# qinzheng93/GeoTransformer

Hardware: NVIDIA H100
Metric: point-cloud pairs/sec (3DMatch-shape synth) (higher is better)
Workload: dtype f32

## Files before the change

__graft_entry__.py:

```python
import os
import subprocess
import sys

ROOT = os.path.dirname(os.path.abspath(__file__))
if ROOT not in sys.path:
    sys.path.insert(0, ROOT)


def build():
    jobs = str(os.cpu_count() or 4)
    subprocess.check_call(['make', '-C', os.path.join(ROOT, 'geotransformer_b200', 'csrc'), '-j', jobs])
    subprocess.check_call(['make', '-C', os.path.join(ROOT, 'oracle'), 'all'])
    from oracle import normals_oracle, voxel_oracle
    voxel_oracle.build()
    normals_oracle.build()
    import geotransformer_b200
    from geotransformer_b200 import _lib
    _lib.lib()


def smoke():
    import numpy as np
    import torch
    from geotransformer_b200.config import make_cfg
    from geotransformer_b200.model import create_model
    from geotransformer_b200.synth import make_pair
    from geotransformer_b200.utils.data import registration_collate_fn_stack_mode
    from geotransformer_b200.weights import synthetic_state_dict
    from oracle import geo_oracle as G

    assert torch.cuda.is_available(), 'smoke() needs a GPU'
    torch.cuda.set_device(0)
    cfg = make_cfg('3dmatch')
    model = create_model(cfg)
    model.load_state_dict(synthetic_state_dict(model, 7351), strict=True)
    model = model.cuda().eval()
    pair = make_pair('demo2k', 0)
    dd = {k: pair[k] for k in ('ref_points', 'src_points', 'ref_feats', 'src_feats', 'transform')}
# ... 50 lines not shown
```

geotransformer_b200/_lib.py:

```python
import ctypes
import os
import threading

import torch

_HERE = os.path.dirname(os.path.abspath(__file__))
LIB_PATH = os.path.join(_HERE, 'libgeob200.so')
_lib = None

c_void_p, c_int64, c_int32, c_float, c_double, c_size_t, c_int = (
    ctypes.c_void_p, ctypes.c_int64, ctypes.c_int32, ctypes.c_float, ctypes.c_double, ctypes.c_size_t, ctypes.c_int)

SIGNATURES = {}


def _sig(name, restype, *argtypes):
    SIGNATURES[name] = (restype, list(argtypes))


P, I64, I32, F, D, SZ = c_void_p, c_int64, c_int32, c_float, c_double, c_size_t
_sig('geob200_last_error', ctypes.c_char_p)
_sig('geob200_launch_count', ctypes.c_uint64)
_sig('geob200_grid_subsample_workspace_bytes', SZ, I64, I64)
_sig('geob200_grid_subsample', c_int, P, I64, P, I64, F, P, P, P, SZ, P)
_sig('geob200_radius_search_workspace_bytes', SZ, I64, I64, I64)
_sig('geob200_radius_search', c_int, P, I64, P, I64, P, P, I64, F, I64, P, P, P, P, SZ, P)

_sig('geob200_neighbor_histogram', c_int, P, I64, I64, I64, I64, P, P)
_sig('geob200_neighbor_histogram_batched', c_int, P, P, P, I64, I64, I64, I64, P, P, P, P)
_sig('geob200_voxel_down_sample_workspace_bytes', SZ, I64, I64)
_sig('geob200_voxel_down_sample', c_int, P, P, I64, P, I64, D, P, P, P, P, SZ, P)
_sig('geob200_estimate_normals_workspace_bytes', SZ, I64, I64)
_sig('geob200_estimate_normals', c_int, P, I64, P, I64, I64, D, P, P, P, P, P, SZ, P)
_sig('geob200_regularize_normals', c_int, P, P, I64, c_int, c_int, P, P)
_sig('geob200_kernel_point_optimize', c_int, P, I64, I64, ctypes.c_uint64, D, P, P, P)
_sig('geob200_kernel_point_instances', c_int, P, I64, P, P, I64, ctypes.c_uint64, P, P)
_sig('geob200_kpconv_workspace_bytes', SZ, I64)
_sig('geob200_kpconv', c_int, P, P, P, P, I64, I64, I64, P, I64, P, P, I64, I64, F, P, P, SZ, P)
_sig('geob200_kpconv_tc_workspace_bytes', SZ, I64, I64, I64)
_sig('geob200_kpconv_tc', c_int, P, P, P, P, I64, I64, I64, P, I64, P, P, I64, I64, F, P, P, SZ, P)
_sig('geob200_set_linear_mode', None, c_int)
_sig('geob200_linear', c_int, P, I64, P, P, P, I64, I64, I64, I64, c_int, P)
_sig('geob200_split_tf32', c_int, P, I64, I64, I64, P, P)
_sig('geob200_linear_batched', c_int, P, I64, I64, P, I64, I64, P, I64, P, I64, I64, I64, I64, I64, I64, c_int, P)
_sig('geob200_group_norm_workspace_bytes', SZ, I64)
_sig('geob200_group_norm', c_int, P, I64, I64, I64, P, P, F, P, c_int, F, P, P, SZ, P)
_sig('geob200_fused_group_norm_workspace_bytes', SZ, I64, I64, I64)
_sig('geob200_linear_group_norm', c_int, P, I64, P, P, I64, I64, I64, I64, P, P, F, P, c_int, F, P, P, P, SZ, P)
_sig('geob200_kpconv_group_norm', c_int, P, P, P, P, I64, I64, I64, P, I64, P, P, I64, I64, F, I64, P, P, F, c_int, F, P, P, P, SZ,
     P, SZ, P)
_sig('geob200_group_norm_batched', c_int, P, I64, I64, I64, P, P, F, P, c_int, F, P, P, SZ, P, I64, P)
_sig('geob200_linear_group_norm_batched', c_int, P, I64, P, P, I64, I64, I64, I64, P, P, F, P, c_int, F, P, P, P, SZ, P, I64, P)
_sig('geob200_maxpool', c_int, P, P, I64, I64, I64, I64, P, P)
_sig('geob200_upsample_concat', c_int, P, P, I64, I64, P, I64, I64, I64, P, P)
_sig('geob200_kpconv_backward_workspace_bytes', SZ, I64, I64, I64, I64, I64)
_sig('geob200_kpconv_backward', c_int, P, P, P, P, I64, I64, I64, P, I64, P, I64, I64, F, P, P, P, P, P, SZ, P)
_sig('geob200_linear_backward_workspace_bytes', SZ, I64, I64, I64, c_int)
_sig('geob200_linear_backward', c_int, P, I64, P, P, I64, I64, I64, P, P, P, P, P, SZ, P)
_sig('geob200_group_norm_backward_batched_workspace_bytes', SZ, I64, I64, I64, I64)
_sig('geob200_group_norm_backward_batched', c_int, P, P, I64, I64, I64, P, F, c_int, F, P, P, P, P, P, P, SZ, P, I64, P)
_sig('geob200_maxpool_backward_batched_workspace_bytes', SZ, I64, I64, I64, I64)
_sig('geob200_maxpool_backward_batched', c_int, P, P, I64, I64, I64, I64, P, I64, P, P, P, P, SZ, P)
_sig('geob200_upsample_concat_backward_workspace_bytes', SZ, I64, I64)
# ... 177 lines not shown
```

geotransformer_b200/csrc/kpconv.cu:

```cuda
#include "common.cuh"
#include "geob200.h"
#include "kpconv.cuh"

namespace geob200 {

constexpr int TQ = 32;
constexpr int CC = 32;

__global__ void __launch_bounds__(256) kpconv_c1_kernel(const float* __restrict__ feats, const float* __restrict__ q_pts,
                                                        const float* __restrict__ s_pts, const long long* __restrict__ nbr,
                                                        int H, const float* __restrict__ kp, const float* __restrict__ W,
                                                        const float* __restrict__ bias, float sigma, int Ns, int M, int Cout,
                                                        float* __restrict__ out) {
    __shared__ float kp_s[KP * 3];
    __shared__ float wk_s[16][KP_PAD];
    __shared__ float np_s[16];
    if (threadIdx.x < KP * 3) kp_s[threadIdx.x] = kp[threadIdx.x];
    __syncthreads();
    const int lane = threadIdx.x & 31, warp = threadIdx.x >> 5;
    const int sub = lane >> 4, sl = lane & 15;
    const int slot = warp * 2 + sub;
    const int m = blockIdx.x * 16 + slot;
    const bool live = m < M;
    float acc[KP];
// ... 28 lines not shown
    }
    __syncwarp();
    if (!live) return;
    for (int c = sl; c < Cout; c += 16) {
        float o = 0.f;
#pragma unroll
        for (int k = 0; k < KP; ++k) o = fmaf(wk_s[slot][k], W[k * Cout + c], o);
        o = o / np_s[slot];
        if (bias != nullptr) o += bias[c];
        out[(long long)m * Cout + c] = o;
    }
}

__global__ void __launch_bounds__(256) row_positive_kernel(const float* __restrict__ x, int N, int C, unsigned char* __restrict__ pos) {
    const int lane = threadIdx.x & 31;
    const int n = blockIdx.x * 8 + (threadIdx.x >> 5);
    if (n >= N) return;
    float s = 0.f;
    for (int c = lane; c < C; c += 32) s += x[(long long)n * C + c];
    s = warp_sum(s);
    if (lane == 0) pos[n] = (s > 0.f) ? 1 : 0;
}

template <int CPL>
__global__ void __launch_bounds__(256, 4) kpconv_gather_kernel(const float* __restrict__ feats, const unsigned char* __restrict__ pos,
                                                            const float* __restrict__ q_pts, const float* __restrict__ s_pts,
                                                            const long long* __restrict__ nbr, int H, const float* __restrict__ kp,
                                                            float sigma, int Ns, int M, int Cin, float* __restrict__ wf,
                                                            float* __restrict__ inv_count) {
    __shared__ float infl[8][32][KP_PAD];
    __shared__ int sidx[8][32];
    __shared__ float kp_s[KP * 3];
    const int lane = threadIdx.x & 31, warp = threadIdx.x >> 5;
    if (threadIdx.x < KP * 3) kp_s[threadIdx.x] = kp[threadIdx.x];
    __syncthreads();
    const int m = blockIdx.x * 8 + warp;
    if (m >= M) return;
    const float qx = q_pts[3ll * m], qy = q_pts[3ll * m + 1], qz = q_pts[3ll * m + 2];
    int npos = 0;
    for (int c0 = 0; c0 < Cin; c0 += 32 * CPL) {
        float acc[CPL][KP];
#pragma unroll
        for (int p = 0; p < CPL; ++p)
#pragma unroll
            for (int k = 0; k < KP; ++k) acc[p][k] = 0.f;
        for (int h0 = 0; h0 < H; h0 += 32) {
            const int h = h0 + lane;
            const long long idx = (h < H) ? nbr[(long long)m * H + h] : (long long)Ns;
            float w[KP];
            int id = 0;
            if (idx < Ns) {
                id = (int)idx;
                influence15(kp_s, s_pts[3 * idx] - qx, s_pts[3 * idx + 1] - qy, s_pts[3 * idx + 2] - qz, 0.f, sigma, w);
                if (c0 == 0) npos += pos[idx];
            } else {
#pragma unroll
                for (int k = 0; k < KP; ++k) w[k] = 0.f;
            }
            __syncwarp();
#pragma unroll
            for (int k = 0; k < KP; ++k) infl[warp][lane][k] = w[k];
            infl[warp][lane][KP] = 0.f;
            sidx[warp][lane] = id;
            __syncwarp();
            const int hn = min(32, H - h0);
            for (int hb = 0; hb < hn; hb += 8) {
                float f[8][CPL];
#pragma unroll
                for (int u = 0; u < 8; ++u)
#pragma unroll
                    for (int p = 0; p < CPL; ++p)
                        f[u][p] = __ldg(feats + (long long)sidx[warp][(hb + u) & 31] * Cin + c0 + 32 * p + lane);
#pragma unroll
                for (int u = 0; u < 8; ++u) {
                    if (hb + u < hn) {
                        const float4* iv = reinterpret_cast<const float4*>(&infl[warp][hb + u][0]);
                        const float4 a0 = iv[0], a1 = iv[1], a2 = iv[2], a3 = iv[3];
                        const float wv[16] = {a0.x, a0.y, a0.z, a0.w, a1.x, a1.y, a1.z, a1.w, a2.x, a2.y, a2.z, a2.w, a3.x, a3.y, a3.z, a3.w};
#pragma unroll
                        for (int p = 0; p < CPL; ++p)
#pragma unroll
                            for (int k = 0; k < KP; ++k) acc[p][k] = fmaf(wv[k], f[u][p], acc[p][k]);
                    }
                }
            }
        }
#pragma unroll
        for (int p = 0; p < CPL; ++p) {
            float* wrow = wf + (long long)m * (KP * Cin) + c0 + 32 * p + lane;
#pragma unroll
            for (int k = 0; k < KP; ++k) wrow[(long long)k * Cin] = acc[p][k];
        }
    }
#pragma unroll
    for (int o = 16; o > 0; o >>= 1) npos += __shfl_xor_sync(0xffffffffu, npos, o);
    if (lane == 0) inv_count[m] = 1.0f / (float)max(npos, 1);
}

static void launch_kpconv_gather(const float* s_feats, const unsigned char* pos, const float* q_points, const float* s_points,
                                 const long long* neighbors, int n_neighbors, const float* kernel_points, float sigma, int n_support,
                                 int n_query, int c_in, float* wf, float* inv_count, cudaStream_t st) {
    const unsigned grid = (unsigned)((n_query + 7) / 8);
    if (c_in % 64 == 0)
        kpconv_gather_kernel<2><<<grid, 256, 0, st>>>(s_feats, pos, q_points, s_points, neighbors, n_neighbors, kernel_points, sigma,
                                                     n_support, n_query, c_in, wf, inv_count);
    else
        kpconv_gather_kernel<1><<<grid, 256, 0, st>>>(s_feats, pos, q_points, s_points, neighbors, n_neighbors, kernel_points, sigma,
                                                     n_support, n_query, c_in, wf, inv_count);
}

void kpconv_gather(const float* s_feats, const float* q_points, const float* s_points, const long long* neighbors, int n_neighbors,
                   const float* kernel_points, float sigma, int n_support, int n_query, int c_in, unsigned char* pos, float* wf,
                   float* inv_count, cudaStream_t st) {
    row_positive_kernel<<<(unsigned)((n_support + 7) / 8), 256, 0, st>>>(s_feats, n_support, c_in, pos);
    launch_kpconv_gather(s_feats, pos, q_points, s_points, neighbors, n_neighbors, kernel_points, sigma, n_support, n_query, c_in, wf,
                         inv_count, st);
    count_launches(2);
}

template <int RC>
__global__ void __launch_bounds__(256) kpconv_kernel(const float* __restrict__ feats, const unsigned char* __restrict__ pos,
                                                     const float* __restrict__ q_pts, const float* __restrict__ s_pts,
                                                     const long long* __restrict__ nbr, int H, const float* __restrict__ kp,
                                                     const float* __restrict__ W, const float* __restrict__ bias, float sigma,
                                                     int Ns, int M, int Cin, int Cout, float* __restrict__ out) {
    const int col0 = blockIdx.y * (RC * 32);
    extern __shared__ float smem[];
    float* wf = smem;
    float* infl = wf + TQ * KP * CC;
    int* sidx = (int*)(infl + 8 * 32 * KP_PAD);
    float* npos_s = (float*)(sidx + 8 * 32);
    float* kp_s = npos_s + TQ;
    const int lane = threadIdx.x & 31, warp = threadIdx.x >> 5;
    if (threadIdx.x < KP * 3) kp_s[threadIdx.x] = kp[threadIdx.x];
    __syncthreads();
    const int m0 = blockIdx.x * TQ;

    float acc_out[4][RC];
#pragma unroll
    for (int r = 0; r < 4; ++r)
// ... 616 lines not shown
    const long long idx = up[(long long)m * up_stride];
    float* yr = y + (long long)m * (C1 + C2);
    for (int c = lane; c < C1; c += 32) yr[c] = (idx < Ns) ? x[idx * C1 + c] : 0.f;
    if (skip != nullptr)
        for (int c = lane; c < C2; c += 32) yr[C1 + c] = skip[(long long)m * C2 + c];
}

}

using namespace geob200;

namespace geob200 {
int linear_tc(const float* x, int64_t ldx, const float* w, int64_t ldw, const float* w_img, const float* bias, const float* row_scale, float* y, int64_t ldy,
              int64_t m, int64_t n, int64_t k, int relu, cudaStream_t st, const GnFuse* gn = nullptr);
static int g_linear_mode = 1;
}

extern "C" {

void geob200_set_linear_mode(int mode) { g_linear_mode = mode; }

size_t geob200_kpconv_workspace_bytes(int64_t n_support) { return (size_t)n_support + 256; }

size_t geob200_kpconv_tc_workspace_bytes(int64_t n_query, int64_t n_support, int64_t c_in) {
    return align_up((size_t)n_support, 256) + align_up((size_t)n_query * 4, 256) + (size_t)n_query * KP * (size_t)c_in * 4 + 1024;
}

int geob200_kpconv_tc(const float* s_feats, const float* q_points, const float* s_points, const int64_t* neighbors, int64_t n_query,
                      int64_t n_support, int64_t n_neighbors, const float* kernel_points, int64_t n_kernel, const float* weights_t,
                      const float* bias, int64_t c_in, int64_t c_out, float sigma, float* out, void* workspace, size_t workspace_bytes,
                      void* stream) {
    return geob200::kpconv_tc_impl(s_feats, q_points, s_points, neighbors, n_query, n_support, n_neighbors, kernel_points, n_kernel,
                                   weights_t, nullptr, bias, c_in, c_out, sigma, out, workspace, workspace_bytes, stream);
}
}

namespace geob200 {
int kpconv_tc_impl(const float* s_feats, const float* q_points, const float* s_points, const int64_t* neighbors, int64_t n_query,
                   int64_t n_support, int64_t n_neighbors, const float* kernel_points, int64_t n_kernel, const float* weights_t,
                   const float* w_img, const float* bias, int64_t c_in, int64_t c_out, float sigma, float* out, void* workspace,
                   size_t workspace_bytes, void* stream) {
    cudaStream_t st = (cudaStream_t)stream;
    GEOB_REQUIRE(n_kernel == KP, "kpconv_tc: kernel_size %lld unsupported", (long long)n_kernel);
    GEOB_REQUIRE(n_query > 0 && n_support > 0 && n_neighbors > 0, "kpconv_tc: empty input");
    GEOB_REQUIRE(c_in % 32 == 0 && c_out % 16 == 0 && c_out >= 32 && (c_out <= 128 || c_out % 128 == 0) && n_query >= 64,
                 "kpconv_tc: unsupported shape (%lld -> %lld, %lld queries)", (long long)c_in, (long long)c_out, (long long)n_query);
    GEOB_REQUIRE(workspace_bytes >= geob200_kpconv_tc_workspace_bytes(n_query, n_support, c_in), "kpconv_tc: workspace too small");
    Arena ar(workspace, workspace_bytes);
    unsigned char* pos = ar.take<unsigned char>(n_support);
    float* inv_count = ar.take<float>(n_query);
    float* wf = ar.take<float>((size_t)n_query * KP * c_in);
    row_positive_kernel<<<(unsigned)((n_support + 7) / 8), 256, 0, st>>>(s_feats, (int)n_support, (int)c_in, pos);
    launch_kpconv_gather(s_feats, pos, q_points, s_points, (const long long*)neighbors, (int)n_neighbors, kernel_points, sigma,
                         (int)n_support, (int)n_query, (int)c_in, wf, inv_count, st);
    GEOB_CHECK_LAUNCH();
    count_launches(2);
    const int rc = linear_tc(wf, KP * c_in, weights_t, KP * c_in, w_img, bias, inv_count, out, c_out, n_query, c_out, KP * c_in, 0, st);
    GEOB_REQUIRE(rc == 0, "kpconv_tc: tensor-core GEMM rejected the shape");
    return 0;
}

int linear_img(const float* x, int64_t ldx, const float* weight, const float* w_img, const float* bias, float* y, int64_t ldy,
               int64_t m, int64_t n, int64_t k, int relu, void* stream) {
    if (g_linear_mode == 1 && m > 0 && n > 0 && k > 0) {
        const int rc = linear_tc(x, ldx, weight, k, w_img, bias, nullptr, y, ldy, m, n, k, relu, (cudaStream_t)stream);
        if (rc <= 0) return rc;
    }
    return geob200_linear(x, ldx, weight, bias, y, ldy, m, n, k, relu, stream);
}
}

extern "C" {

int geob200_kpconv(const float* s_feats, const float* q_points, const float* s_points, const int64_t* neighbors,
                   int64_t n_query, int64_t n_support, int64_t n_neighbors, const float* kernel_points, int64_t n_kernel,
                   const float* weights, const float* bias, int64_t c_in, int64_t c_out, float sigma, float* out,
                   void* workspace, size_t workspace_bytes, void* stream) {
    cudaStream_t st = (cudaStream_t)stream;
    GEOB_REQUIRE(n_kernel == KP, "kpconv: kernel_size %lld unsupported (all shipped models use 15)", (long long)n_kernel);
// ... 248 lines not shown
namespace geob200 {
int kpconv_group_norm_impl(const float* s_feats, const float* q_points, const float* s_points, const int64_t* neighbors,
                           int64_t n_query, int64_t n_support, int64_t n_neighbors, const float* kernel_points, int64_t n_kernel,
                           const float* weights_t, const float* bias, int64_t c_in, int64_t c_out, float sigma, int64_t groups,
                           const float* gamma, const float* beta, float eps, int leaky, float slope, float* pre_norm, float* y,
                           void* gn_workspace, size_t gn_workspace_bytes, void* workspace, size_t workspace_bytes, void* stream,
                           const GnSeg* seg, const float* w_img) {
    cudaStream_t st = (cudaStream_t)stream;
    const int64_t np = (seg != nullptr && seg->n_pairs > 1) ? seg->n_pairs : 1;
    GEOB_REQUIRE(n_kernel == KP, "kpconv_group_norm: kernel_size %lld unsupported", (long long)n_kernel);
    GEOB_REQUIRE(n_query > 0 && n_support > 0 && n_neighbors > 0, "kpconv_group_norm: empty input");
    GEOB_REQUIRE(c_in % 32 == 0 && c_out % 16 == 0 && c_out >= 32 && (c_out <= 128 || c_out % 128 == 0) && n_query >= 64,
                 "kpconv_group_norm: unsupported shape (%lld -> %lld, %lld queries)", (long long)c_in, (long long)c_out,
                 (long long)n_query);
    GEOB_REQUIRE(groups > 0 && c_out % groups == 0, "kpconv_group_norm: bad group count");
    GEOB_REQUIRE(gn_workspace_bytes >= (np > 1 ? fused_group_norm_workspace_bytes_batched(n_query, c_out, groups, np)
                                               : geob200_fused_group_norm_workspace_bytes(n_query, c_out, groups)),
                 "kpconv_group_norm: GroupNorm workspace too small");
    GEOB_REQUIRE(workspace_bytes >= geob200_kpconv_tc_workspace_bytes(n_query, n_support, c_in), "kpconv_group_norm: workspace too small");
    Arena ar(workspace, workspace_bytes);
    unsigned char* pos = ar.take<unsigned char>(n_support);
    float* inv_count = ar.take<float>(n_query);
    float* wf = ar.take<float>((size_t)n_query * KP * c_in);
    row_positive_kernel<<<(unsigned)((n_support + 7) / 8), 256, 0, st>>>(s_feats, (int)n_support, (int)c_in, pos);
    launch_kpconv_gather(s_feats, pos, q_points, s_points, (const long long*)neighbors, (int)n_neighbors, kernel_points, sigma,
                         (int)n_support, (int)n_query, (int)c_in, wf, inv_count, st);
    GEOB_CHECK_LAUNCH();
    count_launches(2);
    const GnWs w = gn_carve(gn_workspace, gn_workspace_bytes, groups, np);
    GnFuse gn{(int)groups, 0, w.partial};
    int rc = linear_tc(wf, KP * c_in, weights_t, KP * c_in, w_img, bias, inv_count, pre_norm, c_out, n_query, c_out, KP * c_in, 0, st, &gn);
    if (rc < 0) return rc;
    if (rc == 0) {
        if (np > 1) {
            launch_gn_seg_apply(pre_norm, w, gamma, beta, nullptr, y, n_query, c_out, groups, eps, leaky, slope, *seg, st);
        } else {
            launch_gn_apply(pre_norm, w, gamma, beta, nullptr, y, n_query, c_out, groups, eps, leaky, slope, st);
            count_launches(2);
        }
        GEOB_CHECK_LAUNCH();
        return 0;
    }
    rc = linear_tc(wf, KP * c_in, weights_t, KP * c_in, w_img, bias, inv_count, pre_norm, c_out, n_query, c_out, KP * c_in, 0, st);
    GEOB_REQUIRE(rc == 0, "kpconv_group_norm: tensor-core GEMM rejected the shape");
    return group_norm_impl(pre_norm, n_query, c_out, groups, gamma, beta, eps, nullptr, leaky, slope, y, gn_workspace, gn_workspace_bytes,
                           stream, seg);
}
}

namespace geob200 {
int make_seg(GnSeg* g, int64_t n_pairs, const int64_t* cloud_rows_h, int64_t n_rows, const char* what) {
// ... 86 lines not shown
```

geotransformer_b200/csrc/kpconv.cuh:

```cuda
#pragma once
#include "common.cuh"

namespace geob200 {

constexpr int KP = 15;
constexpr int KP_PAD = 16;

__device__ __forceinline__ void influence15(const float* __restrict__ kp_s, float rx, float ry, float rz, float inv_dummy,
                                            float sigma, float* w) {
#pragma unroll
    for (int k = 0; k < KP; ++k) {
        const float dx = rx - kp_s[3 * k], dy = ry - kp_s[3 * k + 1], dz = rz - kp_s[3 * k + 2];
        const float sq = __fadd_rn(__fadd_rn(__fmul_rn(dx, dx), __fmul_rn(dy, dy)), __fmul_rn(dz, dz));
        w[k] = fmaxf(1.0f - sqrtf(sq) / sigma, 0.0f);
    }
    (void)inv_dummy;
}

__device__ __forceinline__ int cloud_of(const int* start, int n_clouds, int row) {
    int lo = 0, hi = n_clouds;
    while (hi - lo > 1) {
        const int mid = (lo + hi) >> 1;
        if (start[mid] <= row) lo = mid; else hi = mid;
    }
    return lo;
}

int make_seg(GnSeg* g, int64_t n_pairs, const int64_t* cloud_rows_h, int64_t n_rows, const char* what);

void kpconv_gather(const float* s_feats, const float* q_points, const float* s_points, const long long* neighbors, int n_neighbors,
                   const float* kernel_points, float sigma, int n_support, int n_query, int c_in, unsigned char* pos, float* wf,
                   float* inv_count, cudaStream_t st);

size_t atb_bytes(int64_t M, int64_t ka, int64_t n);
void atb(const float* A, long long lda, const float* B, long long ldb, const float* s, int64_t M, int64_t ka, int64_t n, float* C,
         float* part, cudaStream_t st);

}
```

geotransformer_b200/csrc/kpconv_grad.cu:

```cuda
#include "common.cuh"
#include "geob200.h"
#include "kpconv.cuh"

namespace geob200 {

__global__ void __launch_bounds__(1024) exclusive_scan_kernel(const int* __restrict__ cnt, int n, int* __restrict__ off);

struct IndexTable {
    const long long* idx;
    long long ld;
    int rows, cols, n_support;
    __device__ __forceinline__ int target(int e) const {
        const int m = e / cols, h = e - m * cols;
        const long long v = idx[(long long)m * ld + h];
        return (v >= 0 && v < n_support) ? (int)v : -1;
    }
};

__global__ void __launch_bounds__(256) csr_count_kernel(IndexTable t, int* __restrict__ cnt) {
    const int e = blockIdx.x * blockDim.x + threadIdx.x;
    if (e >= t.rows * t.cols) return;
    const int s = t.target(e);
    if (s >= 0) atomicAdd(&cnt[s], 1);
}
// ... 456 lines not shown
    GEOB_REQUIRE(n_query > 0 && n_support > 0 && n_neighbors > 0 && c_out > 0, "kpconv_backward: empty input");
    GEOB_REQUIRE(c_in == 1 || c_in % 32 == 0, "kpconv_backward: c_in %lld must be 1 or a multiple of 32", (long long)c_in);
    GEOB_REQUIRE(n_query * n_neighbors < (1ll << 31) && n_query * KP * c_in < (1ll << 40), "kpconv_backward: neighbour table too large");
    GEOB_REQUIRE(s_feats != nullptr && q_points != nullptr && s_points != nullptr && neighbors != nullptr && kernel_points != nullptr &&
                 grad_out != nullptr && (grad_feats == nullptr || weights != nullptr), "kpconv_backward: null input");
    GEOB_REQUIRE(workspace != nullptr &&
                 workspace_bytes >= geob200_kpconv_backward_workspace_bytes(n_query, n_support, n_neighbors, c_in, c_out),
                 "kpconv_backward: workspace too small");
    const int64_t ka = KP * c_in;
    Arena ar(workspace, workspace_bytes);
    unsigned char* pos = ar.take<unsigned char>(n_support);
    float* inv_count = ar.take<float>(n_query);
    float* wf = ar.take<float>((size_t)n_query * ka);
    float* part = ar.take<float>(atb_bytes(n_query, ka, c_out) / 4 + atb_bytes(n_query, 1, c_out) / 4 + 1);
    const long long* nbr = (const long long*)neighbors;
    if (grad_bias != nullptr) atb(nullptr, 0, grad_out, c_out, nullptr, n_query, 1, c_out, grad_bias, part, st);
    if (grad_weights != nullptr || grad_feats != nullptr) {
        if (c_in == 1) {
            kpconv_c1_wf_kernel<<<(unsigned)((n_query + 15) / 16), 256, 0, st>>>(s_feats, q_points, s_points, nbr, (int)n_neighbors,
                                                                                 kernel_points, sigma, (int)n_support, (int)n_query, wf,
                                                                                 inv_count);
            count_launches(1);
        } else {
            kpconv_gather(s_feats, q_points, s_points, nbr, (int)n_neighbors, kernel_points, sigma, (int)n_support, (int)n_query, (int)c_in,
                          pos, wf, inv_count, st);
        }
    }
    if (grad_weights != nullptr) atb(wf, ka, grad_out, c_out, inv_count, n_query, ka, c_out, grad_weights, part, st);
    if (grad_feats != nullptr) {
        const int rc = linear_img(grad_out, c_out, weights, nullptr, nullptr, wf, ka, n_query, ka, c_out, 0, stream);
        if (rc != 0) return rc;
        Csr csr;
        const IndexTable t{nbr, n_neighbors, (int)n_query, (int)n_neighbors, (int)n_support};
        if (build_csr(t, ar, &csr, st)) return -1;
        kpconv_dx_kernel<<<(unsigned)((n_support + 7) / 8), 256, 0, st>>>(wf, inv_count, q_points, s_points, kernel_points, sigma,
                                                                          (int)n_neighbors, (int)n_support, (int)c_in, csr.off,
                                                                          csr.sorted, grad_feats);
        count_launches(1);
    }
    GEOB_REQUIRE(ar.ok(), "kpconv_backward: workspace accounting error");
    GEOB_CHECK_LAUNCH();
    return 0;
}

size_t geob200_linear_backward_workspace_bytes(int64_t m, int64_t n, int64_t k, int relu) {
    return atb_bytes(m, n, k) + atb_bytes(m, 1, n) + (relu ? align_up((size_t)m * n * 4, 256) : 0) + 1024;
}

// ... 131 lines not shown
```

geotransformer_b200/functional.py:

```python
import ctypes
import math

import torch

from . import _lib as L

_f32, _i64, _u8, _i32 = torch.float32, torch.int64, torch.uint8, torch.int32

GSE_MODE = 5
GSE_TABLE_INV_STEP = 256
GSE_TABLE_D_MAX = 96.0

EVENTS = None


class _timed:
    def __init__(self, name):
        self.name = name

    def __enter__(self):
        if EVENTS is not None:
            self.s = torch.cuda.Event(enable_timing=True)
            self.e = torch.cuda.Event(enable_timing=True)
            self.s.record()
# ... 47 lines not shown
def _kpconv(s_feats, q_points, s_points, neighbor_indices, kernel_points, weights, bias, sigma, weights_t=None):
    s_feats, weights, bias = _detach(s_feats), _detach(weights), _detach(bias)
    _f(s_feats, 's_feats'); _f(q_points, 'q_points'); _f(s_points, 's_points')
    L.require_cuda(neighbor_indices, 'neighbor_indices', _i64)
    m, h = neighbor_indices.shape
    ns = s_points.shape[0]
    k, cin, cout = weights.shape
    out = torch.empty((m, cout), dtype=_f32, device=s_feats.device)
    lib = L.lib()
    if (KPCONV_MODE == 'tc' and cin % 32 == 0 and cout % 16 == 0 and cout >= 32 and (cout <= 128 or cout % 128 == 0) and m >= 64):
        if weights_t is None:
            weights_t = weights.reshape(k * cin, cout).t().contiguous()
        ws = L.workspace(lib.geob200_kpconv_tc_workspace_bytes(m, ns, cin), s_feats.device, 'kpconv_tc')
        L.check(lib.geob200_kpconv_tc(s_feats.data_ptr(), q_points.data_ptr(), s_points.data_ptr(), neighbor_indices.data_ptr(), m, ns,
                                      h, kernel_points.data_ptr(), k, weights_t.data_ptr(), L.ptr(bias), cin, cout, float(sigma),
                                      out.data_ptr(), ws.data_ptr(), ws.numel(), L.stream_ptr()), 'kpconv_tc')
        return out
    ws = L.workspace(lib.geob200_kpconv_workspace_bytes(ns), s_feats.device, 'kpconv')
    L.check(lib.geob200_kpconv(s_feats.data_ptr(), q_points.data_ptr(), s_points.data_ptr(),
                               neighbor_indices.data_ptr(), m, ns, h, kernel_points.data_ptr(), k,
                               weights.data_ptr(), L.ptr(bias), cin, cout, float(sigma), out.data_ptr(),
                               ws.data_ptr(), ws.numel(), L.stream_ptr()), 'kpconv')
    return out


def kpconv_backward(s_feats, q_points, s_points, neighbor_indices, kernel_points, weights, sigma, grad_out, need_feats=True,
                    need_weights=True, need_bias=True):
    for t, name in ((s_feats, 's_feats'), (q_points, 'q_points'), (s_points, 's_points'), (kernel_points, 'kernel_points'),
                    (weights, 'weights'), (grad_out, 'grad_out')):
        _f(_detach(t), name)
    L.require_cuda(neighbor_indices, 'neighbor_indices', _i64)
    s_feats, weights = _detach(s_feats), _detach(weights)
    m, h = neighbor_indices.shape
    ns = s_points.shape[0]
    k, cin, cout = weights.shape
    if tuple(grad_out.shape) != (m, cout) or tuple(s_feats.shape) != (ns, cin):
        raise RuntimeError(f'kpconv_backward: grad_out must be ({m}, {cout}) and s_feats ({ns}, {cin})')
    dev = s_feats.device
    gf = torch.empty((ns, cin), dtype=_f32, device=dev) if need_feats else None
    gw = torch.empty((k, cin, cout), dtype=_f32, device=dev) if need_weights else None
    gb = torch.empty((cout,), dtype=_f32, device=dev) if need_bias else None
    lib = L.lib()
    ws = L.workspace(lib.geob200_kpconv_backward_workspace_bytes(m, ns, h, cin, cout), dev, 'kpconv_backward')
    L.check(lib.geob200_kpconv_backward(s_feats.data_ptr(), q_points.data_ptr(), s_points.data_ptr(), neighbor_indices.data_ptr(), m, ns, h,
                                        kernel_points.data_ptr(), k, weights.data_ptr(), cin, cout, float(sigma), grad_out.data_ptr(),
                                        L.ptr(gf), L.ptr(gw), L.ptr(gb), ws.data_ptr(), ws.numel(), L.stream_ptr()), 'kpconv_backward')
# ... 2360 lines not shown
```

include/geob200.h:

```cpp
#ifndef GEOB200_H
#define GEOB200_H

#include <stddef.h>
#include <stdint.h>

#ifdef __cplusplus
extern "C" {
#endif

const char* geob200_last_error(void);
uint64_t geob200_launch_count(void);


size_t geob200_grid_subsample_workspace_bytes(int64_t n_points, int64_t batch);
int geob200_grid_subsample(const float* points, int64_t n_points, const int64_t* lengths_h, int64_t batch, float voxel,
                           float* s_points, int64_t* s_lengths, void* workspace, size_t workspace_bytes, void* stream);

size_t geob200_radius_search_workspace_bytes(int64_t n_query, int64_t n_support, int64_t batch);
int geob200_radius_search(const float* q_points, int64_t n_query, const float* s_points, int64_t n_support,
                          const int64_t* q_lengths_h, const int64_t* s_lengths_h, int64_t batch, float radius,
                          int64_t width, int64_t* out, int32_t* counts, int32_t* max_count, void* workspace,
                          size_t workspace_bytes, void* stream);

int geob200_neighbor_histogram(const int64_t* neighbors, int64_t n_rows, int64_t width, int64_t n_support, int64_t hist_n,
// ... 24 lines not shown
                             size_t workspace_bytes, void* stream);
int geob200_regularize_normals(const void* points, const void* normals, int64_t n, int fp64, int positive, double* out, void* stream);


#define GEOB200_KP_MAX_POINTS 30
int geob200_kernel_point_optimize(const double* init, int64_t num_kernels, int64_t num_points, uint64_t seed, double ratio,
                                  double* points, int32_t* info, void* stream);

int geob200_kernel_point_instances(const double* disposition, int64_t num_points, const double* radii, const int64_t* layer_ids,
                                   int64_t num_layers, uint64_t seed, float* out, void* stream);


size_t geob200_kpconv_workspace_bytes(int64_t n_support);
int geob200_kpconv(const float* s_feats, const float* q_points, const float* s_points, const int64_t* neighbors,
                   int64_t n_query, int64_t n_support, int64_t n_neighbors, const float* kernel_points, int64_t n_kernel,
                   const float* weights, const float* bias, int64_t c_in, int64_t c_out, float sigma, float* out,
                   void* workspace, size_t workspace_bytes, void* stream);

size_t geob200_kpconv_tc_workspace_bytes(int64_t n_query, int64_t n_support, int64_t c_in);
int geob200_kpconv_tc(const float* s_feats, const float* q_points, const float* s_points, const int64_t* neighbors, int64_t n_query,
                      int64_t n_support, int64_t n_neighbors, const float* kernel_points, int64_t n_kernel, const float* weights_t,
                      const float* bias, int64_t c_in, int64_t c_out, float sigma, float* out, void* workspace, size_t workspace_bytes,
                      void* stream);

int geob200_split_tf32(const float* w, int64_t ld, int64_t n, int64_t k, float* out, void* stream);

void geob200_set_linear_mode(int mode);
int geob200_linear(const float* x, int64_t ldx, const float* weight, const float* bias, float* y, int64_t ldy, int64_t m,
                   int64_t n, int64_t k, int relu, void* stream);
int geob200_linear_batched(const float* x, int64_t ldx, int64_t stride_x, const float* weight, int64_t ldw, int64_t stride_w,
                           const float* bias, int64_t stride_b, float* y, int64_t ldy, int64_t stride_y, int64_t m, int64_t n,
                           int64_t k, int64_t batch, int relu, void* stream);

size_t geob200_group_norm_workspace_bytes(int64_t groups);
int geob200_group_norm(const float* x, int64_t n_rows, int64_t channels, int64_t groups, const float* gamma,
                       const float* beta, float eps, const float* residual, int leaky, float slope, float* y,
                       void* workspace, size_t workspace_bytes, void* stream);

size_t geob200_fused_group_norm_workspace_bytes(int64_t n_rows, int64_t channels, int64_t groups);
int geob200_linear_group_norm(const float* x, int64_t ldx, const float* weight, const float* bias, int64_t m, int64_t n, int64_t k,
                              int64_t groups, const float* gamma, const float* beta, float eps, const float* residual, int leaky,
                              float slope, float* pre_norm, float* y, void* workspace, size_t workspace_bytes, void* stream);
int geob200_kpconv_group_norm(const float* s_feats, const float* q_points, const float* s_points, const int64_t* neighbors,
                              int64_t n_query, int64_t n_support, int64_t n_neighbors, const float* kernel_points, int64_t n_kernel,
                              const float* weights_t, const float* bias, int64_t c_in, int64_t c_out, float sigma, int64_t groups,
                              const float* gamma, const float* beta, float eps, int leaky, float slope, float* pre_norm, float* y,
// ... 373 lines not shown
```

Measured before the change: 434.7.

## Restructure KPConv gather to pack multiple queries per block with vectorized channel loads

Rewrites the KPConv neighbour-gather kernel. Each 128-thread block now handles several query points, and each thread owns 2 or 4 channels with float2/float4 feature loads, where before one warp handled each query with scalar per-lane loads. Neighbour influence weights are computed cooperatively for the whole block and staged in dynamic shared memory, and the positive-neighbour count is kept with shared atomics. The aim is better memory coalescing and more independent loads in flight for small channel counts. In exchange there are block-wide syncs per neighbour chunk, 15×CPT accumulators per thread that raise register pressure, and new alignment and c_in limits.

Result: no change. 441.6 (median of 6 runs) (+1.6%).

```diff
diff --git a/__graft_entry__.py b/__graft_entry__.py
--- a/__graft_entry__.py
+++ b/__graft_entry__.py
@@ -11,9 +11,10 @@
     jobs = str(os.cpu_count() or 4)
     subprocess.check_call(['make', '-C', os.path.join(ROOT, 'geotransformer_b200', 'csrc'), '-j', jobs])
     subprocess.check_call(['make', '-C', os.path.join(ROOT, 'oracle'), 'all'])
-    from oracle import normals_oracle, voxel_oracle
+    from oracle import kpconv_gather_oracle, normals_oracle, voxel_oracle
     voxel_oracle.build()
     normals_oracle.build()
+    kpconv_gather_oracle.build()
     import geotransformer_b200
     from geotransformer_b200 import _lib
     _lib.lib()
diff --git a/geotransformer_b200/_lib.py b/geotransformer_b200/_lib.py
--- a/geotransformer_b200/_lib.py
+++ b/geotransformer_b200/_lib.py
@@ -39,6 +39,7 @@
 _sig('geob200_kpconv', c_int, P, P, P, P, I64, I64, I64, P, I64, P, P, I64, I64, F, P, P, SZ, P)
 _sig('geob200_kpconv_tc_workspace_bytes', SZ, I64, I64, I64)
 _sig('geob200_kpconv_tc', c_int, P, P, P, P, I64, I64, I64, P, I64, P, P, I64, I64, F, P, P, SZ, P)
+_sig('geob200_kpconv_gather', c_int, P, P, P, P, I64, I64, I64, P, I64, I64, F, P, P, P, SZ, P)
 _sig('geob200_set_linear_mode', None, c_int)
 _sig('geob200_linear', c_int, P, I64, P, P, P, I64, I64, I64, I64, c_int, P)
 _sig('geob200_split_tf32', c_int, P, I64, I64, I64, P, P)
diff --git a/geotransformer_b200/csrc/kpconv.cu b/geotransformer_b200/csrc/kpconv.cu
--- a/geotransformer_b200/csrc/kpconv.cu
+++ b/geotransformer_b200/csrc/kpconv.cu
@@ -1,3 +1,5 @@
+#include <type_traits>
+
 #include "common.cuh"
 #include "geob200.h"
 #include "kpconv.cuh"
@@ -74,100 +76,138 @@
     if (lane == 0) pos[n] = (s > 0.f) ? 1 : 0;
 }
 
-template <int CPL>
-__global__ void __launch_bounds__(256, 4) kpconv_gather_kernel(const float* __restrict__ feats, const unsigned char* __restrict__ pos,
-                                                            const float* __restrict__ q_pts, const float* __restrict__ s_pts,
-                                                            const long long* __restrict__ nbr, int H, const float* __restrict__ kp,
-                                                            float sigma, int Ns, int M, int Cin, float* __restrict__ wf,
-                                                            float* __restrict__ inv_count) {
-    __shared__ float infl[8][32][KP_PAD];
-    __shared__ int sidx[8][32];
-    __shared__ float kp_s[KP * 3];
-    const int lane = threadIdx.x & 31, warp = threadIdx.x >> 5;
-    if (threadIdx.x < KP * 3) kp_s[threadIdx.x] = kp[threadIdx.x];
+constexpr int GATHER_NB = 32;
+constexpr int GATHER_ROW = GATHER_NB * KP_PAD + 4;
+constexpr int GATHER_U = 8;
+
+template <int CPT>
+__global__ void __launch_bounds__(128, CPT == 4 ? 4 : 6)
+    kpconv_gather_kernel(const float* __restrict__ feats, const unsigned char* __restrict__ pos, const float* __restrict__ q_pts,
+                         const float* __restrict__ s_pts, const long long* __restrict__ nbr, int H, const float* __restrict__ kp,
+                         float sigma, int Ns, int M, int Cin, int G, int QPB, float* __restrict__ wf, float* __restrict__ inv_count) {
+    static_assert(CPT == 2 || CPT == 4, "2 or 4 channels per thread");
+    using Vec = typename std::conditional<CPT == 4, float4, float2>::type;
+    constexpr int GATHER_PPT = CPT;
+    extern __shared__ float4 gather_smem[];
+    float* infl = reinterpret_cast<float*>(gather_smem);
+    int* sidx = reinterpret_cast<int*>(infl + QPB * GATHER_ROW);
+    int* npos_s = sidx + QPB * GATHER_NB;
+    float* kp_s = reinterpret_cast<float*>(npos_s + QPB);
+    const int t = threadIdx.x, nt = blockDim.x;
+    if (t < KP * 3) kp_s[t] = kp[t];
+    if (t < QPB) npos_s[t] = 0;
+    const int q = t / G, g = t - q * G;
+    const int m0 = blockIdx.x * QPB, m = m0 + q;
+    const float* irow = infl + q * GATHER_ROW;
+    const int* ids = sidx + q * GATHER_NB;
+    const float* fcol = feats + CPT * g;
+    float acc[KP][CPT];
+#pragma unroll
+    for (int k = 0; k < KP; ++k)
+#pragma unroll
+        for (int c = 0; c < CPT; ++c) acc[k][c] = 0.f;
     __syncthreads();
-    const int m = blockIdx.x * 8 + warp;
-    if (m >= M) return;
-    const float qx = q_pts[3ll * m], qy = q_pts[3ll * m + 1], qz = q_pts[3ll * m + 2];
-    int npos = 0;
-    for (int c0 = 0; c0 < Cin; c0 += 32 * CPL) {
-        float acc[CPL][KP];
-#pragma unroll
-        for (int p = 0; p < CPL; ++p)
-#pragma unroll
-            for (int k = 0; k < KP; ++k) acc[p][k] = 0.f;
-        for (int h0 = 0; h0 < H; h0 += 32) {
-            const int h = h0 + lane;
-            const long long idx = (h < H) ? nbr[(long long)m * H + h] : (long long)Ns;
+    for (int h0 = 0; h0 < H; h0 += GATHER_NB) {
+        const int hn = min(GATHER_NB, H - h0);
+        long long idx[GATHER_PPT];
+#pragma unroll
+        for (int i = 0; i < GATHER_PPT; ++i) {
+            const int p = t + i * nt, pq = p / hn, j = p - pq * hn;
+            idx[i] = (p < QPB * hn && m0 + pq < M) ? nbr[(long long)(m0 + pq) * H + h0 + j] : (long long)Ns;
+        }
+        float rx[GATHER_PPT], ry[GATHER_PPT], rz[GATHER_PPT];
+        int pv[GATHER_PPT];
+#pragma unroll
+        for (int i = 0; i < GATHER_PPT; ++i) {
+            const long long pm = m0 + (t + i * nt) / hn;
+            rx[i] = ry[i] = rz[i] = 0.f;
+            pv[i] = 0;
+            if (idx[i] < Ns) {
+                rx[i] = s_pts[3 * idx[i]] - q_pts[3 * pm];
+                ry[i] = s_pts[3 * idx[i] + 1] - q_pts[3 * pm + 1];
+                rz[i] = s_pts[3 * idx[i] + 2] - q_pts[3 * pm + 2];
+                pv[i] = pos[idx[i]];
+            }
+        }
+#pragma unroll
+        for (int i = 0; i < GATHER_PPT; ++i) {
+            const int p = t + i * nt, pq = p / hn, j = p - pq * hn;
+            if (p >= QPB * hn) break;
             float w[KP];
             int id = 0;
-            if (idx < Ns) {
-                id = (int)idx;
-                influence15(kp_s, s_pts[3 * idx] - qx, s_pts[3 * idx + 1] - qy, s_pts[3 * idx + 2] - qz, 0.f, sigma, w);
-                if (c0 == 0) npos += pos[idx];
+            if (idx[i] < Ns) {
+                id = (int)idx[i];
+                influence15(kp_s, rx[i], ry[i], rz[i], 0.f, sigma, w);
+                if (pv[i]) atomicAdd(&npos_s[pq], 1);
             } else {
 #pragma unroll
                 for (int k = 0; k < KP; ++k) w[k] = 0.f;
             }
-            __syncwarp();
-#pragma unroll
-            for (int k = 0; k < KP; ++k) infl[warp][lane][k] = w[k];
-            infl[warp][lane][KP] = 0.f;
-            sidx[warp][lane] = id;
-            __syncwarp();
-            const int hn = min(32, H - h0);
-            for (int hb = 0; hb < hn; hb += 8) {
-                float f[8][CPL];
-#pragma unroll
-                for (int u = 0; u < 8; ++u)
-#pragma unroll
-                    for (int p = 0; p < CPL; ++p)
-                        f[u][p] = __ldg(feats + (long long)sidx[warp][(hb + u) & 31] * Cin + c0 + 32 * p + lane);
-#pragma unroll
-                for (int u = 0; u < 8; ++u) {
-                    if (hb + u < hn) {
-                        const float4* iv = reinterpret_cast<const float4*>(&infl[warp][hb + u][0]);
+            float4* row = reinterpret_cast<float4*>(infl + pq * GATHER_ROW + j * KP_PAD);
+            row[0] = make_float4(w[0], w[1], w[2], w[3]);
+            row[1] = make_float4(w[4], w[5], w[6], w[7]);
+            row[2] = make_float4(w[8], w[9], w[10], w[11]);
+            row[3] = make_float4(w[12], w[13], w[14], 0.f);
+            sidx[pq * GATHER_NB + j] = id;
+        }
+        __syncthreads();
+        if (m < M) {
+            for (int j0 = 0; j0 < hn; j0 += GATHER_U) {
+                float f[GATHER_U][CPT];
+#pragma unroll
+                for (int u = 0; u < GATHER_U; ++u) {
+                    const Vec v = __ldg(reinterpret_cast<const Vec*>(fcol + (long long)(j0 + u < hn ? ids[j0 + u] : 0) * Cin));
+#pragma unroll
+                    for (int c = 0; c < CPT; ++c) f[u][c] = reinterpret_cast<const float*>(&v)[c];
+                }
+#pragma unroll
+                for (int u = 0; u < GATHER_U; ++u) {
+                    if (j0 + u < hn) {
+                        const float4* iv = reinterpret_cast<const float4*>(irow + (j0 + u) * KP_PAD);
                         const float4 a0 = iv[0], a1 = iv[1], a2 = iv[2], a3 = iv[3];
-                        const float wv[16] = {a0.x, a0.y, a0.z, a0.w, a1.x, a1.y, a1.z, a1.w, a2.x, a2.y, a2.z, a2.w, a3.x, a3.y, a3.z, a3.w};
-#pragma unroll
-                        for (int p = 0; p < CPL; ++p)
-#pragma unroll
-                            for (int k = 0; k < KP; ++k) acc[p][k] = fmaf(wv[k], f[u][p], acc[p][k]);
+                        const float wv[KP] = {a0.x, a0.y, a0.z, a0.w, a1.x, a1.y, a1.z, a1.w, a2.x, a2.y, a2.z, a2.w, a3.x, a3.y, a3.z};
+#pragma unroll
+                        for (int k = 0; k < KP; ++k)
+#pragma unroll
+                            for (int c = 0; c < CPT; ++c) acc[k][c] = fmaf(wv[k], f[u][c], acc[k][c]);
                     }
                 }
             }
         }
-#pragma unroll
-        for (int p = 0; p < CPL; ++p) {
-            float* wrow = wf + (long long)m * (KP * Cin) + c0 + 32 * p + lane;
-#pragma unroll
-            for (int k = 0; k < KP; ++k) wrow[(long long)k * Cin] = acc[p][k];
-        }
-    }
-#pragma unroll
-    for (int o = 16; o > 0; o >>= 1) npos += __shfl_xor_sync(0xffffffffu, npos, o);
-    if (lane == 0) inv_count[m] = 1.0f / (float)max(npos, 1);
-}
-
-static void launch_kpconv_gather(const float* s_feats, const unsigned char* pos, const float* q_points, const float* s_points,
-                                 const long long* neighbors, int n_neighbors, const float* kernel_points, float sigma, int n_support,
-                                 int n_query, int c_in, float* wf, float* inv_count, cudaStream_t st) {
-    const unsigned grid = (unsigned)((n_query + 7) / 8);
-    if (c_in % 64 == 0)
-        kpconv_gather_kernel<2><<<grid, 256, 0, st>>>(s_feats, pos, q_points, s_points, neighbors, n_neighbors, kernel_points, sigma,
-                                                     n_support, n_query, c_in, wf, inv_count);
+        __syncthreads();
+    }
+    if (m >= M) return;
+    float* wrow = wf + (long long)m * (KP * Cin) + CPT * g;
+#pragma unroll
+    for (int k = 0; k < KP; ++k) {
+        Vec v;
+#pragma unroll
+        for (int c = 0; c < CPT; ++c) reinterpret_cast<float*>(&v)[c] = acc[k][c];
+        *reinterpret_cast<Vec*>(wrow + (long long)k * Cin) = v;
+    }
+    if (g == 0) inv_count[m] = 1.0f / (float)max(npos_s[q], 1);
+}
+
+int kpconv_gather(const float* s_feats, const float* q_points, const float* s_points, const long long* neighbors, int n_neighbors,
+                  const float* kernel_points, float sigma, int n_support, int n_query, int c_in, unsigned char* pos, float* wf,
+                  float* inv_count, cudaStream_t st) {
+    GEOB_REQUIRE(c_in % 32 == 0 && c_in <= 512, "kpconv_gather: c_in %d must be a multiple of 32 and <= 512", c_in);
+    GEOB_REQUIRE(((uintptr_t)s_feats & 15) == 0 && ((uintptr_t)wf & 15) == 0, "kpconv_gather: s_feats and wf must be 16-byte aligned");
+    const int cpt = c_in == 32 ? 2 : 4;
+    const int G = c_in / cpt;
+    const int qpb = 128 / G;
+    const size_t smem = (size_t)qpb * (GATHER_ROW * sizeof(float) + GATHER_NB * sizeof(int) + sizeof(int)) + KP * 3 * sizeof(float);
+    const dim3 grid((unsigned)((n_query + qpb - 1) / qpb)), block((unsigned)(qpb * G));
+    row_positive_kernel<<<(unsigned)((n_support + 7) / 8), 256, 0, st>>>(s_feats, n_support, c_in, pos);
+    if (cpt == 2)
+        kpconv_gather_kernel<2><<<grid, block, smem, st>>>(s_feats, pos, q_points, s_points, neighbors, n_neighbors, kernel_points, sigma,
+                                                          n_support, n_query, c_in, G, qpb, wf, inv_count);
     else
-        kpconv_gather_kernel<1><<<grid, 256, 0, st>>>(s_feats, pos, q_points, s_points, neighbors, n_neighbors, kernel_points, sigma,
-                                                     n_support, n_query, c_in, wf, inv_count);
-}
-
-void kpconv_gather(const float* s_feats, const float* q_points, const float* s_points, const long long* neighbors, int n_neighbors,
-                   const float* kernel_points, float sigma, int n_support, int n_query, int c_in, unsigned char* pos, float* wf,
-                   float* inv_count, cudaStream_t st) {
-    row_positive_kernel<<<(unsigned)((n_support + 7) / 8), 256, 0, st>>>(s_feats, n_support, c_in, pos);
-    launch_kpconv_gather(s_feats, pos, q_points, s_points, neighbors, n_neighbors, kernel_points, sigma, n_support, n_query, c_in, wf,
-                         inv_count, st);
+        kpconv_gather_kernel<4><<<grid, block, smem, st>>>(s_feats, pos, q_points, s_points, neighbors, n_neighbors, kernel_points, sigma,
+                                                          n_support, n_query, c_in, G, qpb, wf, inv_count);
+    GEOB_CHECK_LAUNCH();
     count_launches(2);
+    return 0;
 }
 
 template <int RC>
@@ -830,6 +870,17 @@
 
 size_t geob200_kpconv_workspace_bytes(int64_t n_support) { return (size_t)n_support + 256; }
 
+int geob200_kpconv_gather(const float* s_feats, const float* q_points, const float* s_points, const int64_t* neighbors, int64_t n_query,
+                          int64_t n_support, int64_t n_neighbors, const float* kernel_points, int64_t n_kernel, int64_t c_in, float sigma,
+                          float* wf, float* inv_count, void* workspace, size_t workspace_bytes, void* stream) {
+    GEOB_REQUIRE(n_kernel == KP, "kpconv_gather: kernel_size %lld unsupported", (long long)n_kernel);
+    GEOB_REQUIRE(n_query > 0 && n_support > 0 && n_neighbors > 0, "kpconv_gather: empty input");
+    GEOB_REQUIRE(n_query * n_neighbors < (1ll << 31) && n_support < (1ll << 31), "kpconv_gather: neighbour table too large");
+    GEOB_REQUIRE(workspace != nullptr && workspace_bytes >= geob200_kpconv_workspace_bytes(n_support), "kpconv_gather: workspace too small");
+    return kpconv_gather(s_feats, q_points, s_points, (const long long*)neighbors, (int)n_neighbors, kernel_points, sigma, (int)n_support,
+                         (int)n_query, (int)c_in, (unsigned char*)workspace, wf, inv_count, (cudaStream_t)stream);
+}
+
 size_t geob200_kpconv_tc_workspace_bytes(int64_t n_query, int64_t n_support, int64_t c_in) {
     return align_up((size_t)n_support, 256) + align_up((size_t)n_query * 4, 256) + (size_t)n_query * KP * (size_t)c_in * 4 + 1024;
 }
@@ -858,11 +909,9 @@
     unsigned char* pos = ar.take<unsigned char>(n_support);
     float* inv_count = ar.take<float>(n_query);
     float* wf = ar.take<float>((size_t)n_query * KP * c_in);
-    row_positive_kernel<<<(unsigned)((n_support + 7) / 8), 256, 0, st>>>(s_feats, (int)n_support, (int)c_in, pos);
-    launch_kpconv_gather(s_feats, pos, q_points, s_points, (const long long*)neighbors, (int)n_neighbors, kernel_points, sigma,
-                         (int)n_support, (int)n_query, (int)c_in, wf, inv_count, st);
-    GEOB_CHECK_LAUNCH();
-    count_launches(2);
+    const int grc = kpconv_gather(s_feats, q_points, s_points, (const long long*)neighbors, (int)n_neighbors, kernel_points, sigma,
+                                  (int)n_support, (int)n_query, (int)c_in, pos, wf, inv_count, st);
+    if (grc != 0) return grc;
     const int rc = linear_tc(wf, KP * c_in, weights_t, KP * c_in, w_img, bias, inv_count, out, c_out, n_query, c_out, KP * c_in, 0, st);
     GEOB_REQUIRE(rc == 0, "kpconv_tc: tensor-core GEMM rejected the shape");
     return 0;
@@ -1157,11 +1206,9 @@
     unsigned char* pos = ar.take<unsigned char>(n_support);
     float* inv_count = ar.take<float>(n_query);
     float* wf = ar.take<float>((size_t)n_query * KP * c_in);
-    row_positive_kernel<<<(unsigned)((n_support + 7) / 8), 256, 0, st>>>(s_feats, (int)n_support, (int)c_in, pos);
-    launch_kpconv_gather(s_feats, pos, q_points, s_points, (const long long*)neighbors, (int)n_neighbors, kernel_points, sigma,
-                         (int)n_support, (int)n_query, (int)c_in, wf, inv_count, st);
-    GEOB_CHECK_LAUNCH();
-    count_launches(2);
+    const int grc = kpconv_gather(s_feats, q_points, s_points, (const long long*)neighbors, (int)n_neighbors, kernel_points, sigma,
+                                  (int)n_support, (int)n_query, (int)c_in, pos, wf, inv_count, st);
+    if (grc != 0) return grc;
     const GnWs w = gn_carve(gn_workspace, gn_workspace_bytes, groups, np);
     GnFuse gn{(int)groups, 0, w.partial};
     int rc = linear_tc(wf, KP * c_in, weights_t, KP * c_in, w_img, bias, inv_count, pre_norm, c_out, n_query, c_out, KP * c_in, 0, st, &gn);
diff --git a/geotransformer_b200/csrc/kpconv.cuh b/geotransformer_b200/csrc/kpconv.cuh
--- a/geotransformer_b200/csrc/kpconv.cuh
+++ b/geotransformer_b200/csrc/kpconv.cuh
@@ -28,9 +28,9 @@
 
 int make_seg(GnSeg* g, int64_t n_pairs, const int64_t* cloud_rows_h, int64_t n_rows, const char* what);
 
-void kpconv_gather(const float* s_feats, const float* q_points, const float* s_points, const long long* neighbors, int n_neighbors,
-                   const float* kernel_points, float sigma, int n_support, int n_query, int c_in, unsigned char* pos, float* wf,
-                   float* inv_count, cudaStream_t st);
+int kpconv_gather(const float* s_feats, const float* q_points, const float* s_points, const long long* neighbors, int n_neighbors,
+                  const float* kernel_points, float sigma, int n_support, int n_query, int c_in, unsigned char* pos, float* wf,
+                  float* inv_count, cudaStream_t st);
 
 size_t atb_bytes(int64_t M, int64_t ka, int64_t n);
 void atb(const float* A, long long lda, const float* B, long long ldb, const float* s, int64_t M, int64_t ka, int64_t n, float* C,
diff --git a/geotransformer_b200/csrc/kpconv_grad.cu b/geotransformer_b200/csrc/kpconv_grad.cu
--- a/geotransformer_b200/csrc/kpconv_grad.cu
+++ b/geotransformer_b200/csrc/kpconv_grad.cu
@@ -502,8 +502,9 @@
                                                                                  inv_count);
             count_launches(1);
         } else {
-            kpconv_gather(s_feats, q_points, s_points, nbr, (int)n_neighbors, kernel_points, sigma, (int)n_support, (int)n_query, (int)c_in,
-                          pos, wf, inv_count, st);
+            const int rc = kpconv_gather(s_feats, q_points, s_points, nbr, (int)n_neighbors, kernel_points, sigma, (int)n_support,
+                                         (int)n_query, (int)c_in, pos, wf, inv_count, st);
+            if (rc != 0) return rc;
         }
     }
     if (grad_weights != nullptr) atb(wf, ka, grad_out, c_out, inv_count, n_query, ka, c_out, grad_weights, part, st);
diff --git a/geotransformer_b200/functional.py b/geotransformer_b200/functional.py
--- a/geotransformer_b200/functional.py
+++ b/geotransformer_b200/functional.py
@@ -93,6 +93,23 @@
                                weights.data_ptr(), L.ptr(bias), cin, cout, float(sigma), out.data_ptr(),
                                ws.data_ptr(), ws.numel(), L.stream_ptr()), 'kpconv')
     return out
+
+
+def kpconv_gather(s_feats, q_points, s_points, neighbor_indices, kernel_points, sigma):
+    s_feats = _detach(s_feats)
+    _f(s_feats, 's_feats'); _f(q_points, 'q_points'); _f(s_points, 's_points'); _f(kernel_points, 'kernel_points')
+    L.require_cuda(neighbor_indices, 'neighbor_indices', _i64)
+    m, h = neighbor_indices.shape
+    ns, cin = s_feats.shape
+    dev = s_feats.device
+    wf = torch.empty((m, kernel_points.shape[0] * cin), dtype=_f32, device=dev)
+    inv_count = torch.empty((m,), dtype=_f32, device=dev)
+    lib = L.lib()
+    ws = L.workspace(lib.geob200_kpconv_workspace_bytes(ns), dev, 'kpconv')
+    L.check(lib.geob200_kpconv_gather(s_feats.data_ptr(), q_points.data_ptr(), s_points.data_ptr(), neighbor_indices.data_ptr(), m, ns, h,
+                                      kernel_points.data_ptr(), kernel_points.shape[0], cin, float(sigma), wf.data_ptr(),
+                                      inv_count.data_ptr(), ws.data_ptr(), ws.numel(), L.stream_ptr()), 'kpconv_gather')
+    return wf, inv_count
 
 
 def kpconv_backward(s_feats, q_points, s_points, neighbor_indices, kernel_points, weights, sigma, grad_out, need_feats=True,
diff --git a/include/geob200.h b/include/geob200.h
--- a/include/geob200.h
+++ b/include/geob200.h
@@ -70,6 +70,10 @@
                       int64_t n_support, int64_t n_neighbors, const float* kernel_points, int64_t n_kernel, const float* weights_t,
                       const float* bias, int64_t c_in, int64_t c_out, float sigma, float* out, void* workspace, size_t workspace_bytes,
                       void* stream);
+
+int geob200_kpconv_gather(const float* s_feats, const float* q_points, const float* s_points, const int64_t* neighbors, int64_t n_query,
+                          int64_t n_support, int64_t n_neighbors, const float* kernel_points, int64_t n_kernel, int64_t c_in, float sigma,
+                          float* wf, float* inv_count, void* workspace, size_t workspace_bytes, void* stream);
 
 int geob200_split_tf32(const float* w, int64_t ld, int64_t n, int64_t k, float* out, void* stream);
 
diff --git a/oracle/kpconv_gather_oracle.cpp b/oracle/kpconv_gather_oracle.cpp
--- /dev/null
+++ b/oracle/kpconv_gather_oracle.cpp
@@ -0,0 +1,66 @@
+#include <cmath>
+#include <cstdint>
+#include <vector>
+
+namespace {
+
+bool row_positive(const float* row, int64_t c_in) {
+    float v[32];
+    for (int l = 0; l < 32; ++l) {
+        float s = 0.f;
+        for (int64_t c = l; c < c_in; c += 32) s = s + row[c];
+        v[l] = s;
+    }
+    for (int o = 16; o > 0; o >>= 1) {
+        float nv[32];
+        for (int l = 0; l < 32; ++l) nv[l] = v[l] + v[l ^ o];
+        for (int l = 0; l < 32; ++l) v[l] = nv[l];
+    }
+    return v[0] > 0.f;
+}
+
+}
+
+extern "C" int kpconv_gather_oracle(const float* s_feats, const float* q_points, const float* s_points, const int64_t* neighbors,
+                                    int64_t n_query, int64_t n_support, int64_t n_neighbors, const float* kernel_points, int64_t c_in,
+                                    float sigma, const int64_t* rows, int64_t n_rows, float* wf, float* inv_count) {
+    const int KP = 15;
+    if (n_query <= 0 || n_support <= 0 || n_neighbors <= 0 || c_in <= 0 || n_rows < 0) return 1;
+    std::vector<unsigned char> pos(n_support);
+    for (int64_t n = 0; n < n_support; ++n) pos[n] = row_positive(s_feats + n * c_in, c_in) ? 1 : 0;
+    std::vector<float> w(KP);
+    for (int64_t r = 0; r < n_rows; ++r) {
+        const int64_t m = rows != nullptr ? rows[r] : r;
+        if (m < 0 || m >= n_query) return 1;
+        float* acc = wf + r * KP * c_in;
+        for (int64_t i = 0; i < KP * c_in; ++i) acc[i] = 0.f;
+        int npos = 0;
+        for (int64_t h = 0; h < n_neighbors; ++h) {
+            const int64_t idx = neighbors[m * n_neighbors + h];
+            int64_t row = 0;
+            if (idx < n_support) {
+                if (idx < 0) return 1;
+                row = idx;
+                const float rx = s_points[3 * idx] - q_points[3 * m];
+                const float ry = s_points[3 * idx + 1] - q_points[3 * m + 1];
+                const float rz = s_points[3 * idx + 2] - q_points[3 * m + 2];
+                for (int k = 0; k < KP; ++k) {
+                    const float dx = rx - kernel_points[3 * k], dy = ry - kernel_points[3 * k + 1], dz = rz - kernel_points[3 * k + 2];
+                    const float dxx = dx * dx, dyy = dy * dy, dzz = dz * dz;
+                    const float sq = (dxx + dyy) + dzz;
+                    const float d = sqrtf(sq);
+                    const float q = d / sigma;
+                    w[k] = fmaxf(1.0f - q, 0.0f);
+                }
+                npos += pos[idx];
+            } else {
+                for (int k = 0; k < KP; ++k) w[k] = 0.f;
+            }
+            const float* f = s_feats + row * c_in;
+            for (int k = 0; k < KP; ++k)
+                for (int64_t c = 0; c < c_in; ++c) acc[k * c_in + c] = std::fmaf(w[k], f[c], acc[k * c_in + c]);
+        }
+        inv_count[r] = 1.0f / (float)(npos > 1 ? npos : 1);
+    }
+    return 0;
+}
diff --git a/oracle/kpconv_gather_oracle.py b/oracle/kpconv_gather_oracle.py
--- /dev/null
+++ b/oracle/kpconv_gather_oracle.py
@@ -0,0 +1,51 @@
+import ctypes
+import os
+import subprocess
+
+import numpy as np
+
+_HERE = os.path.dirname(os.path.abspath(__file__))
+SRC = os.path.join(_HERE, 'kpconv_gather_oracle.cpp')
+LIB_PATH = os.path.join(_HERE, 'liboracle_kpconv_gather.so')
+_LIB = None
+
+
+def build():
+    cxx = os.environ.get('CXX', 'g++')
+    if os.path.exists(LIB_PATH) and os.path.getmtime(LIB_PATH) >= os.path.getmtime(SRC):
+        return LIB_PATH
+    subprocess.check_call([cxx, '-O2', '-std=c++17', '-fPIC', '-shared', '-ffp-contract=off', '-o', LIB_PATH, SRC])
+    return LIB_PATH
+
+
+def _lib():
+    global _LIB
+    if _LIB is None:
+        if not os.path.exists(LIB_PATH):
+            build()
+        lib = ctypes.CDLL(LIB_PATH)
+        P, I64 = ctypes.c_void_p, ctypes.c_int64
+        lib.kpconv_gather_oracle.restype = ctypes.c_int
+        lib.kpconv_gather_oracle.argtypes = [P, P, P, P, I64, I64, I64, P, I64, ctypes.c_float, P, I64, P, P]
+        _LIB = lib
+    return _LIB
+
+
+def kpconv_gather(s_feats, q_points, s_points, neighbors, kernel_points, sigma, rows=None):
+    f = np.ascontiguousarray(s_feats, dtype=np.float32)
+    q = np.ascontiguousarray(q_points, dtype=np.float32)
+    s = np.ascontiguousarray(s_points, dtype=np.float32)
+    nbr = np.ascontiguousarray(neighbors, dtype=np.int64)
+    kp = np.ascontiguousarray(kernel_points, dtype=np.float32)
+    assert kp.shape == (15, 3), kp.shape
+    n_query, h = nbr.shape
+    n_support, c_in = f.shape
+    r = None if rows is None else np.ascontiguousarray(rows, dtype=np.int64).reshape(-1)
+    n_rows = n_query if r is None else r.shape[0]
+    wf = np.empty((n_rows, 15 * c_in), dtype=np.float32)
+    inv = np.empty((n_rows,), dtype=np.float32)
+    rc = _lib().kpconv_gather_oracle(f.ctypes.data, q.ctypes.data, s.ctypes.data, nbr.ctypes.data, n_query, n_support, h, kp.ctypes.data,
+                                     c_in, float(sigma), None if r is None else r.ctypes.data, n_rows, wf.ctypes.data, inv.ctypes.data)
+    if rc != 0:
+        raise ValueError(f'kpconv_gather_oracle: error {rc}')
+    return wf, inv
```
